# nihaomiao/CVPR23_LFDM

Measured on AMD Instinct MI355X. Metric: 40-frame 128x128 videos/sec (DDIM-100), higher is better.
Workload: dtype f32; 1 GPU; MUG 128x128, 40-frame DDIM-100 sample, batch=1 per GPU (BASELINE.json configs[1]); global_batch=1, frames=40, latent=32, image=128, sampler=DDIM-100 eta=1, cond_scale=1, parallelism=replicas x1 (videos sharded, no collective)

## Files before the change

cvpr23_lfdm_amd/csrc/attn_lowres.hip:

```cpp
#include <stdlib.h>

#include "attn_core.h"
#include "../../include/lfdm_hip.h"

namespace {

constexpr int NQ = 3 * DH;
constexpr int LDQ = NQ + 4;

template <int NT, int D>
__device__ __forceinline__ void project_wave_d(const float* __restrict__ x, int ldx, int64_t row0, int64_t rstride, int nrows,
                                               int c_begin, int c_end, const float* __restrict__ wf, int C, int head,
                                               f32x4 (&acc)[NT][6], float (&s1)[NT], float (&s2)[NT]) {
  const int lane = threadIdx.x & 63, l15 = lane & 15, ks = lane >> 4;
  const float* arow[NT];
#pragma unroll
  for (int ti = 0; ti < NT; ++ti) {
    int r = 16 * ti + l15;
    if (r >= nrows) r = nrows - 1;
    arow[ti] = x + (row0 + (int64_t)r * rstride) * ldx + 4 * ks;
    s1[ti] = s2[ti] = 0.f;
  }
  const float* brow[6];
#pragma unroll
  for (int nj = 0; nj < 6; ++nj) {
    const int gcol = (nj >> 1) * OUT_LD + head * DH + (nj & 1) * 16 + l15;
    brow[nj] = wf + (int64_t)gcol * C + 4 * ks;
#pragma unroll
    for (int ti = 0; ti < NT; ++ti) acc[ti][nj] = (f32x4){0.f, 0.f, 0.f, 0.f};
  }
  float4 ra[D][NT], rb[D][6];
  const int last = c_end - 16;
#pragma unroll
  for (int d = 0; d < D; ++d) {
    const int c = c_begin + 16 * d < last ? c_begin + 16 * d : last;
#pragma unroll
    for (int ti = 0; ti < NT; ++ti) ra[d][ti] = *reinterpret_cast<const float4*>(arow[ti] + c);
#pragma unroll
    for (int nj = 0; nj < 6; ++nj) rb[d][nj] = *reinterpret_cast<const float4*>(brow[nj] + c);
  }
  for (int c0 = c_begin; c0 < c_end; c0 += 16 * D) {
#pragma unroll
    for (int d = 0; d < D; ++d) {
      float4 a[NT], b[6];
#pragma unroll
      for (int ti = 0; ti < NT; ++ti) a[ti] = ra[d][ti];
#pragma unroll
      for (int nj = 0; nj < 6; ++nj) b[nj] = rb[d][nj];
      const int cn = c0 + 16 * (d + D) < last ? c0 + 16 * (d + D) : last;
#pragma unroll
      for (int ti = 0; ti < NT; ++ti) ra[d][ti] = *reinterpret_cast<const float4*>(arow[ti] + cn);
#pragma unroll
      for (int nj = 0; nj < 6; ++nj) rb[d][nj] = *reinterpret_cast<const float4*>(brow[nj] + cn);
#pragma unroll
      for (int ti = 0; ti < NT; ++ti) {
        s1[ti] += (a[ti].x + a[ti].y) + (a[ti].z + a[ti].w);
        s2[ti] += (a[ti].x * a[ti].x + a[ti].y * a[ti].y) + (a[ti].z * a[ti].z + a[ti].w * a[ti].w);
      }
#pragma unroll
      for (int nj = 0; nj < 6; ++nj)
#pragma unroll
        for (int ti = 0; ti < NT; ++ti) {
          acc[ti][nj] = mfma_16x16x4(a[ti].x, b[nj].x, acc[ti][nj]);
          acc[ti][nj] = mfma_16x16x4(a[ti].y, b[nj].y, acc[ti][nj]);
          acc[ti][nj] = mfma_16x16x4(a[ti].z, b[nj].z, acc[ti][nj]);
          acc[ti][nj] = mfma_16x16x4(a[ti].w, b[nj].w, acc[ti][nj]);
        }
    }
  }
#pragma unroll
  for (int ti = 0; ti < NT; ++ti) {
    s1[ti] += __shfl_xor(s1[ti], 16); s2[ti] += __shfl_xor(s2[ti], 16);
    s1[ti] += __shfl_xor(s1[ti], 32); s2[ti] += __shfl_xor(s2[ti], 32);
  }
}

template <int NT, int G, int D>
__device__ __forceinline__ void project_wave_asm(const float* __restrict__ x, int ldx, int64_t row0, int64_t rstride, int nrows,
                                                 int c_begin, const float* __restrict__ wf, int C, int head,
                                                 f32x4 (&acc)[NT][6], float (&s1)[NT], float (&s2)[NT]) {
  const int lane = threadIdx.x & 63, l15 = lane & 15, ks = lane >> 4;
  const float* arow[NT];
#pragma unroll
  for (int ti = 0; ti < NT; ++ti) {
    int r = 16 * ti + l15;
    if (r >= nrows) r = nrows - 1;
    arow[ti] = x + (row0 + (int64_t)r * rstride) * ldx + c_begin + 4 * ks;
    s1[ti] = s2[ti] = 0.f;
  }
  const float* brow[6];
#pragma unroll
  for (int nj = 0; nj < 6; ++nj) {
    const int gcol = (nj >> 1) * OUT_LD + head * DH + (nj & 1) * 16 + l15;
    brow[nj] = wf + (int64_t)gcol * C + c_begin + 4 * ks;
#pragma unroll
    for (int ti = 0; ti < NT; ++ti) acc[ti][nj] = (f32x4){0.f, 0.f, 0.f, 0.f};
  }
  f32x4 ra[D][NT], rb[D][6];
  auto issue = [&](auto gc) {
    constexpr int g = decltype(gc)::value, st = g % D;
    lfdm_static_for<0, NT>([&](auto ti) { lfdm_gload_f4<64 * g>(ra[st][decltype(ti)::value], arow[decltype(ti)::value]); });
    lfdm_static_for<0, 6>([&](auto nj) { lfdm_gload_f4<64 * g>(rb[st][decltype(nj)::value], brow[decltype(nj)::value]); });
  };
  lfdm_static_for<0, (D < G ? D : G)>(issue);
  lfdm_static_for<0, G>([&](auto gc) {
    constexpr int g = decltype(gc)::value, st = g % D;
    constexpr int younger = (G - 1 - g) < (D - 1) ? (G - 1 - g) : (D - 1);
    lfdm_vmwait<younger * (NT + 6)>();
#pragma unroll
    for (int ti = 0; ti < NT; ++ti) lfdm_tie(ra[st][ti]);
#pragma unroll
    for (int nj = 0; nj < 6; ++nj) lfdm_tie(rb[st][nj]);
    f32x4 a[NT], b[6];
#pragma unroll
    for (int ti = 0; ti < NT; ++ti) a[ti] = ra[st][ti];
#pragma unroll
    for (int nj = 0; nj < 6; ++nj) b[nj] = rb[st][nj];
    if constexpr (NT <= 2 && g + D < G) issue(std::integral_constant<int, g + D>{});
#pragma unroll
    for (int ti = 0; ti < NT; ++ti) {
      s1[ti] += (a[ti][0] + a[ti][1]) + (a[ti][2] + a[ti][3]);
      s2[ti] += (a[ti][0] * a[ti][0] + a[ti][1] * a[ti][1]) + (a[ti][2] * a[ti][2] + a[ti][3] * a[ti][3]);
    }
#pragma unroll
    for (int e = 0; e < 4; ++e)
#pragma unroll
      for (int nj = 0; nj < 6; ++nj)
#pragma unroll
        for (int ti = 0; ti < NT; ++ti) acc[ti][nj] = mfma_16x16x4(a[ti][e], b[nj][e], acc[ti][nj]);
    if constexpr (NT > 2 && g + D < G) issue(std::integral_constant<int, g + D>{});
  });
#pragma unroll
  for (int ti = 0; ti < NT; ++ti) {
    s1[ti] += __shfl_xor(s1[ti], 16); s2[ti] += __shfl_xor(s2[ti], 16);
    s1[ti] += __shfl_xor(s1[ti], 32); s2[ti] += __shfl_xor(s2[ti], 32);
  }
}

template <int NT, bool ASM = true>
__device__ __forceinline__ void project_wave(const float* __restrict__ x, int ldx, int64_t row0, int64_t rstride, int nrows,
                                             int c_begin, int c_end, const float* __restrict__ wf, int C, int head,
                                             f32x4 (&acc)[NT][6], float (&s1)[NT], float (&s2)[NT]) {
  const int groups = ASM ? (c_end - c_begin) >> 4 : 0;
  constexpr int D = NT == 1 ? 4 : 2;
  if (groups == 8) project_wave_asm<NT, 8, D>(x, ldx, row0, rstride, nrows, c_begin, wf, C, head, acc, s1, s2);
  else if (groups == 4) project_wave_asm<NT, 4, D>(x, ldx, row0, rstride, nrows, c_begin, wf, C, head, acc, s1, s2);
  else if (groups == 2) project_wave_asm<NT, 2, 2>(x, ldx, row0, rstride, nrows, c_begin, wf, C, head, acc, s1, s2);
  else project_wave_d<NT, 1>(x, ldx, row0, rstride, nrows, c_begin, c_end, wf, C, head, acc, s1, s2);
}

template <int NT, bool ASM = true>
__device__ __forceinline__ void project_ksplit(const float* __restrict__ x, int ldx, int64_t row0, int64_t rstride, int nrows,
                                               const float* __restrict__ wf, int C, int head, float eps, float* part,
                                               float* pstat, float* wsl, float wsum_val) {
  constexpr int R = 16 * NT;
  const int tid = threadIdx.x, lane = tid & 63, wave = tid >> 6, l15 = lane & 15, ks = lane >> 4;
  f32x4 acc[NT][6];
  float s1[NT], s2[NT];
  const int cw = C / 4;
  project_wave<NT, ASM>(x, ldx, row0, rstride, nrows, wave * cw, (wave + 1) * cw, wf, C, head, acc, s1, s2);
  float* mine = part + wave * (R * LDQ);
  if (tid < NQ) wsl[tid] = wsum_val;
#pragma unroll
  for (int ti = 0; ti < NT; ++ti) {
    if (ks == 0) {
      pstat[(0 * 4 + wave) * R + 16 * ti + l15] = s1[ti];
      pstat[(1 * 4 + wave) * R + 16 * ti + l15] = s2[ti];
    }
#pragma unroll
    for (int nj = 0; nj < 6; ++nj)
#pragma unroll
      for (int r = 0; r < 4; ++r) mine[(16 * ti + 4 * ks + r) * LDQ + 16 * nj + l15] = acc[ti][nj][r];
  }
  __syncthreads();
  const float inv_c = 1.0f / (float)C;
  for (int it = tid; it < R * (NQ / 4); it += 256) {
    const int row = it / (NQ / 4), q4 = it - row * (NQ / 4);
    float sv = 0.f, qv = 0.f;
#pragma unroll
    for (int w = 0; w < 4; ++w) {
      sv += pstat[(0 * 4 + w) * R + row];
      qv += pstat[(1 * 4 + w) * R + row];
    }
    const float mean = sv * inv_c;
    float var = qv * inv_c - mean * mean;
    if (var < 0.f) var = 0.f;
    const float rstd = 1.0f / sqrtf(var + eps);
    float4 v = *reinterpret_cast<const float4*>(part + row * LDQ + 4 * q4);
#pragma unroll
    for (int w = 1; w < 4; ++w) {
      const float4 u = *reinterpret_cast<const float4*>(part + w * (R * LDQ) + row * LDQ + 4 * q4);
      v.x += u.x; v.y += u.y; v.z += u.z; v.w += u.w;
    }
    const float4 ws = *reinterpret_cast<const float4*>(wsl + 4 * q4);
    v.x = rstd * (v.x - mean * ws.x); v.y = rstd * (v.y - mean * ws.y);
    v.z = rstd * (v.z - mean * ws.z); v.w = rstd * (v.w - mean * ws.w);
    *reinterpret_cast<float4*>(part + row * LDQ + 4 * q4) = v;
  }
  __syncthreads();
}

__device__ __forceinline__ float load_wsum(const float* __restrict__ wsum, int head) {
  const int tid = threadIdx.x;
  return tid < NQ ? wsum[(tid >> 5) * OUT_LD + head * DH + (tid & 31)] : 0.f;
}

template <int NT, bool MSPLIT>
__global__ __launch_bounds__(256) void linattn_lowres_kernel(const float* __restrict__ x, int ldx, int C,
                                                             const float* __restrict__ wf, const float* __restrict__ wsum,
                                                             float* __restrict__ out, int hw, float eps) {
  constexpr int R = 16 * NT;
  constexpr int ROWS = MSPLIT ? 4 * R : R;
  __shared__ __attribute__((aligned(16))) float qkv[(MSPLIT ? ROWS : 4 * R) * LDQ];
  __shared__ float pstat[2 * 4 * R];
  __shared__ __attribute__((aligned(16))) float wsl[NQ];
  __shared__ float red[8][DH], kmax[DH], ksum[DH];
  __shared__ __attribute__((aligned(16))) float ctx[DH][DH + 4];
  const int tid = threadIdx.x, lane = tid & 63, wave = tid >> 6, l15 = lane & 15, ks = lane >> 4;
  const int f = blockIdx.x >> 3, head = blockIdx.x & 7;
  const int64_t row0 = (int64_t)f * hw;
  const float wsum_val = load_wsum(wsum, head);

  if (MSPLIT) {
    f32x4 acc[NT][6];
    float s1[NT], s2[NT];
    const int nrows_w = hw - wave * R;
    project_wave<NT>(x, ldx, row0 + wave * R, 1, nrows_w < R ? nrows_w : R, 0, C, wf, C, head, acc, s1, s2);
    if (tid < NQ) wsl[tid] = wsum_val;
    if (ks == 0) {
#pragma unroll
      for (int ti = 0; ti < NT; ++ti) {
        const float mean = s1[ti] / (float)C;
        float var = s2[ti] / (float)C - mean * mean;
        if (var < 0.f) var = 0.f;
        pstat[wave * R + 16 * ti + l15] = mean;
        pstat[4 * R + wave * R + 16 * ti + l15] = 1.0f / sqrtf(var + eps);
      }
    }
    __syncthreads();
#pragma unroll
    for (int ti = 0; ti < NT; ++ti)
#pragma unroll
      for (int r = 0; r < 4; ++r) {
        const int rl = 16 * ti + 4 * ks + r;
        const float mean = pstat[wave * R + rl], rstd = pstat[4 * R + wave * R + rl];
#pragma unroll
        for (int nj = 0; nj < 6; ++nj)
          qkv[(wave * R + rl) * LDQ + 16 * nj + l15] = rstd * (acc[ti][nj][r] - mean * wsl[16 * nj + l15]);
      }
    __syncthreads();
  } else {
    project_ksplit<NT>(x, ldx, row0, 1, hw, wf, C, head, eps, qkv, pstat, wsl, wsum_val);
  }

  {
    const int d = tid & 31, part = tid >> 5;
    float m = -3.0e38f;
    for (int n = part; n < hw; n += 8) m = fmaxf(m, qkv[n * LDQ + DH + d]);
    red[part][d] = m;
    __syncthreads();
    if (tid < DH) {
      float mm = red[0][tid];
#pragma unroll
      for (int p = 1; p < 8; ++p) mm = fmaxf(mm, red[p][tid]);
      kmax[tid] = mm;
    }
    __syncthreads();
    const float mx = kmax[d];
    float s = 0.f;
    for (int n = part; n < hw; n += 8) {
      const float e = fast_exp(qkv[n * LDQ + DH + d] - mx);
      qkv[n * LDQ + DH + d] = e;
      s += e;
    }
    red[part][d] = s;
    __syncthreads();
    if (tid < DH) {
      float ss = 0.f;
#pragma unroll
      for (int p = 0; p < 8; ++p) ss += red[p][tid];
      ksum[tid] = ss;
    }
    __syncthreads();
  }
  {
    const int d = tid >> 3, e0 = (tid & 7) * 4;
    float a0 = 0.f, a1 = 0.f, a2 = 0.f, a3 = 0.f;
    for (int n = 0; n < hw; ++n) {
      const float e = qkv[n * LDQ + DH + d];
      const float4 v4 = *reinterpret_cast<const float4*>(qkv + n * LDQ + 2 * DH + e0);
      a0 = fmaf(e, v4.x, a0); a1 = fmaf(e, v4.y, a1); a2 = fmaf(e, v4.z, a2); a3 = fmaf(e, v4.w, a3);
    }
    const float ss = fast_rcp(ksum[d]);
    *reinterpret_cast<float4*>(&ctx[d][e0]) = make_float4(a0 * ss, a1 * ss, a2 * ss, a3 * ss);
  }
  for (int n0 = 0; n0 < hw; n0 += 32) {
    const bool live = n0 + (tid >> 3) < hw;
    const int n = live ? n0 + (tid >> 3) : hw - 1;
    float4 q4 = *reinterpret_cast<const float4*>(qkv + n * LDQ + 4 * (tid & 7));
    float m = fmaxf(fmaxf(q4.x, q4.y), fmaxf(q4.z, q4.w));
    m = fmaxf(m, __shfl_xor(m, 1)); m = fmaxf(m, __shfl_xor(m, 2)); m = fmaxf(m, __shfl_xor(m, 4));
    q4.x = fast_exp(q4.x - m); q4.y = fast_exp(q4.y - m); q4.z = fast_exp(q4.z - m); q4.w = fast_exp(q4.w - m);
    float s = (q4.x + q4.y) + (q4.z + q4.w);
    s += __shfl_xor(s, 1); s += __shfl_xor(s, 2); s += __shfl_xor(s, 4);
    s = ATT_SCALE * fast_rcp(s);
    q4.x *= s; q4.y *= s; q4.z *= s; q4.w *= s;
    if (live) *reinterpret_cast<float4*>(qkv + n * LDQ + 4 * (tid & 7)) = q4;
  }
  __syncthreads();
  for (int it = tid; it < hw * 8; it += 256) {
    const int n = it >> 3, e0 = (it & 7) * 4;
    float4 o = make_float4(0.f, 0.f, 0.f, 0.f);
#pragma unroll
    for (int d4 = 0; d4 < DH / 4; ++d4) {
      const float4 q4 = *reinterpret_cast<const float4*>(qkv + n * LDQ + 4 * d4);
      const float qd[4] = {q4.x, q4.y, q4.z, q4.w};
#pragma unroll
      for (int i = 0; i < 4; ++i) {
        const float4 c4 = *reinterpret_cast<const float4*>(&ctx[4 * d4 + i][e0]);
        o.x = fmaf(c4.x, qd[i], o.x); o.y = fmaf(c4.y, qd[i], o.y); o.z = fmaf(c4.z, qd[i], o.z); o.w = fmaf(c4.w, qd[i], o.w);
      }
    }
    *reinterpret_cast<float4*>(out + (row0 + n) * OUT_LD + head * DH + e0) = o;
  }
}

template <int NT>
__global__ __launch_bounds__(256) void attn_lowres_kernel(const float* __restrict__ x, int ldx, int C,
                                                          const float* __restrict__ wf, const float* __restrict__ wsum,
                                                          float* __restrict__ out, int frames, int hw, int mode,
                                                          const float* __restrict__ bias, const float* __restrict__ rot_cos,
                                                          const float* __restrict__ rot_sin, float eps) {
  constexpr int R = 16 * NT;
  __shared__ __attribute__((aligned(16))) float qkv[4 * R * LDQ];
  __shared__ float pstat[2 * 4 * R];
  __shared__ __attribute__((aligned(16))) float wsl[NQ];
  const int tid = threadIdx.x, lane = tid & 63, wave = tid >> 6, l15 = lane & 15, lq = lane >> 4;
  const int64_t unit = blockIdx.x;
  const int64_t seq = unit >> 3;
  const int head = (int)(unit & 7);
  int64_t row0, tstride;
  seq_rows(seq, mode, frames, hw, row0, tstride);
  const int L = mode == 0 ? frames : hw;
  const float wsum_val = load_wsum(wsum, head);
  project_ksplit<NT, (NT <= 3)>(x, ldx, row0, tstride, L, wf, C, head, eps, qkv, pstat, wsl, wsum_val);

  for (int ti = wave; ti < NT; ti += 4) {
    float qf[8], kf[NT][8];
    {
      const int t = ti * 16 + l15;
      const float* src = qkv + t * LDQ + 8 * lq;
      const float4 q0 = *reinterpret_cast<const float4*>(src), q1 = *reinterpret_cast<const float4*>(src + 4);
      qf[0] = q0.x * ATT_SCALE; qf[1] = q0.y * ATT_SCALE; qf[2] = q0.z * ATT_SCALE; qf[3] = q0.w * ATT_SCALE;
      qf[4] = q1.x * ATT_SCALE; qf[5] = q1.y * ATT_SCALE; qf[6] = q1.z * ATT_SCALE; qf[7] = q1.w * ATT_SCALE;
      if (rot_cos && t < L) {
#pragma unroll
        for (int pr = 0; pr < 4; ++pr) {
          const float c = rot_cos[t * 16 + 4 * lq + pr], sn = rot_sin[t * 16 + 4 * lq + pr];
          rot_pair(qf[2 * pr], qf[2 * pr + 1], c, sn);
        }
      }
    }
#pragma unroll
    for (int tj = 0; tj < NT; ++tj) {
      const int t = tj * 16 + l15;
      const float* src = qkv + t * LDQ + DH + 8 * lq;
      const float4 k0 = *reinterpret_cast<const float4*>(src), k1 = *reinterpret_cast<const float4*>(src + 4);
      kf[tj][0] = k0.x; kf[tj][1] = k0.y; kf[tj][2] = k0.z; kf[tj][3] = k0.w;
      kf[tj][4] = k1.x; kf[tj][5] = k1.y; kf[tj][6] = k1.z; kf[tj][7] = k1.w;
      if (rot_cos && t < L) {
#pragma unroll
        for (int pr = 0; pr < 4; ++pr) {
          const float c = rot_cos[t * 16 + 4 * lq + pr], sn = rot_sin[t * 16 + 4 * lq + pr];
          rot_pair(kf[tj][2 * pr], kf[tj][2 * pr + 1], c, sn);
        }
      }
    }
    f32x4 st[NT];
#pragma unroll
    for (int tj = 0; tj < NT; ++tj) {
      f32x4 a = {0.f, 0.f, 0.f, 0.f};
#pragma unroll
      for (int s = 0; s < 8; ++s) a = mfma_16x16x4(kf[tj][s], qf[s], a);
      st[tj] = a;
    }
    const float inv = softmax_tile<NT, true>(st, head, L, ti * 16 + l15, lq, bias, false);
    f32x4 o0 = {0.f, 0.f, 0.f, 0.f}, o1 = o0;
#pragma unroll
    for (int tj = 0; tj < NT; ++tj)
#pragma unroll
      for (int r = 0; r < 4; ++r) {
        const float p = st[tj][r] * inv;
        const float* vr = qkv + (16 * tj + 4 * lq + r) * LDQ + 2 * DH;
        o0 = mfma_16x16x4(p, vr[l15], o0);
        o1 = mfma_16x16x4(p, vr[16 + l15], o1);
      }
#pragma unroll
    for (int r = 0; r < 4; ++r) {
      const int t = ti * 16 + lq * 4 + r;
      if (t < L) {
        float* dst = out + (row0 + (int64_t)t * tstride) * OUT_LD + head * DH;
        dst[l15] = o0[r];
        dst[16 + l15] = o1[r];
      }
    }
  }
}

bool lowres_args_ok(const float* x, int ldx, int channels, const float* wqkv, const float* wsum, const float* out) {
  return x && wqkv && wsum && out && channels >= 64 && channels % 64 == 0 && ldx >= channels && ldx % 4 == 0 &&
         ((((uintptr_t)x) | ((uintptr_t)wqkv) | ((uintptr_t)out)) & 15) == 0;
}

}

extern "C" int lfdm_linear_attention_lowres_cl_f32(const float* x, int ldx, int channels, const float* wqkv, const float* wsum,
                                                   float* out, int n_frames, int hw, float ln_eps, lfdm_stream_t stream_) {
  hipStream_t stream = (hipStream_t)stream_;
  if (!lowres_args_ok(x, ldx, channels, wqkv, wsum, out) || n_frames <= 0 || hw <= 0 || hw > 256 || (int64_t)n_frames * HEADS > 0x7fffffff) {
    lfdm_set_error("linear_attention_lowres: needs C % 64 == 0, 1 <= hw <= 256 pixels per frame, 16-byte aligned rows");
    return LFDM_EINVAL;
  }
  const dim3 grid((unsigned)(n_frames * HEADS)), block(256);
  if (hw > 192) LFDM_LAUNCH((linattn_lowres_kernel<4, true>), grid, block, 0, stream, x, ldx, channels, wqkv, wsum, out, hw, ln_eps);
  else if (hw > 64) {
    lfdm_set_error("linear_attention_lowres: 64 < hw <= 192 pixels per frame is not built (use the unfused entry points)");
    return LFDM_EINVAL;
  } else
    lfdm_ladder<16, 32, 64>(hw, [&](auto rows) {
      LFDM_LAUNCH((linattn_lowres_kernel<decltype(rows)::value / 16, false>), grid, block, 0, stream, x, ldx, channels, wqkv, wsum, out, hw, ln_eps);
    });
  return lfdm_check_launch("linear_attention_lowres");
}

extern "C" int lfdm_attention_lowres_cl_f32(const float* x, int ldx, int channels, const float* wqkv, const float* wsum,
                                            float* out, int batch, int frames, int hw, int mode, const float* bias,
                                            const float* rot_cos, const float* rot_sin, float ln_eps, lfdm_stream_t stream_) {
  hipStream_t stream = (hipStream_t)stream_;
  const int L = mode == 0 ? frames : hw;
  const int64_t nseq = mode == 0 ? (int64_t)batch * hw : (int64_t)batch * frames;
  if (!lowres_args_ok(x, ldx, channels, wqkv, wsum, out) || batch <= 0 || frames <= 0 || hw <= 0 || (mode != 0 && mode != 1) || L > 64 ||
      ((rot_cos == nullptr) != (rot_sin == nullptr)) || nseq * HEADS > 0x7fffffff) {
    lfdm_set_error("attention_lowres: needs C % 64 == 0, <= 64 tokens per sequence, 16-byte aligned rows");
    return LFDM_EINVAL;
  }
  const dim3 grid((unsigned)(nseq * HEADS)), block(256);
  lp_ladder(L, [&](auto lp) {
    LFDM_LAUNCH((attn_lowres_kernel<decltype(lp)::value / 16>), grid, block, 0, stream, x, ldx, channels, wqkv, wsum, out, frames, hw, mode, bias, rot_cos, rot_sin, ln_eps);
  });
  return lfdm_check_launch("attention_lowres");
}
```

cvpr23_lfdm_amd/csrc/lfdm_device.h:

```cpp
#pragma once
#include <stddef.h>
#include <stdint.h>
#include <type_traits>

#if defined(LFDM_EMU_BUILD)
#include "hip_emu.h"
typedef emu_f32x16 f32x16;
typedef emu_f32x4 f32x4;
#define LFDM_LAUNCH(kern, grid, block, smem, stream, ...) \
  emu::launch(grid, block, smem, [=]() { kern(__VA_ARGS__); })
static inline f32x16 mfma_32x32x2(float a, float b, f32x16 c) { return emu_mfma_32x32x2(a, b, c); }
static inline f32x4 mfma_16x16x4(float a, float b, f32x4 c) { return emu_mfma_16x16x4(a, b, c); }
static inline f32x4 mfma_4x4x1(float a, float b, f32x4 c) { return emu_mfma_4x4x1(a, b, c); }
struct lfdm_bf16x8 { uint16_t h[8]; };
static inline uint16_t lfdm_f32_to_bf16(float f) {
  uint32_t u;
  memcpy(&u, &f, 4);
  if ((u & 0x7fffffffu) > 0x7f800000u) return (uint16_t)((u >> 16) | 0x40u);
  u += 0x7fffu + ((u >> 16) & 1u);
  return (uint16_t)(u >> 16);
}
static inline float lfdm_bf16_to_f32(uint16_t h) {
  const uint32_t u = (uint32_t)h << 16;
  float f;
  memcpy(&f, &u, 4);
  return f;
}
static inline lfdm_bf16x8 lfdm_cvt_bf16x8(float4 a0, float4 a1) {
  const float f[8] = {a0.x, a0.y, a0.z, a0.w, a1.x, a1.y, a1.z, a1.w};
  lfdm_bf16x8 r;
  for (int i = 0; i < 8; ++i) r.h[i] = lfdm_f32_to_bf16(f[i]);
  return r;
}
static inline uint32_t lfdm_cvt_pk_bf16(float lo, float hi) { return (uint32_t)lfdm_f32_to_bf16(lo) | ((uint32_t)lfdm_f32_to_bf16(hi) << 16); }
static inline lfdm_bf16x8 lfdm_bf16x8_bits(float4 v) {
  lfdm_bf16x8 r;
  memcpy(&r, &v, 16);
  return r;
}
static inline f32x16 mfma_32x32x16_bf16(lfdm_bf16x8 a, lfdm_bf16x8 b, f32x16 c) {
  struct Pair { lfdm_bf16x8 a, b; };
  struct Whole { lfdm_bf16x8 a[2], b[2]; };
  const unsigned lane = emu::lane_id(), h = lane >> 5;
  const Pair other = emu::wave_read_from(Pair{a, b}, lane ^ 32u);
  Whole mine;
  mine.a[h] = a;
  mine.a[1 - h] = other.a;
  mine.b[h] = b;
  mine.b[1 - h] = other.b;
  for (int r = 0; r < 16; ++r) {
    const unsigned row = (r & 3) + 8 * (r >> 2) + 4 * h;
    const Whole src = emu::wave_read_from(mine, row);
    float acc = c[r];
    for (int k = 0; k < 16; ++k)
      acc = fmaf(lfdm_bf16_to_f32(src.a[k >> 3].h[k & 7]), lfdm_bf16_to_f32(mine.b[k >> 3].h[k & 7]), acc);
    c[r] = acc;
  }
  return c;
}
#else
#include <hip/hip_runtime.h>
typedef float f32x16 __attribute__((ext_vector_type(16)));
typedef float f32x4 __attribute__((ext_vector_type(4)));
#define LFDM_LAUNCH(kern, grid, block, smem, stream, ...) \
  hipLaunchKernelGGL(kern, grid, block, smem, stream, __VA_ARGS__)
__device__ __forceinline__ f32x16 mfma_32x32x2(float a, float b, f32x16 c) {
  return __builtin_amdgcn_mfma_f32_32x32x2f32(a, b, c, 0, 0, 0);
}
__device__ __forceinline__ f32x4 mfma_16x16x4(float a, float b, f32x4 c) {
  return __builtin_amdgcn_mfma_f32_16x16x4f32(a, b, c, 0, 0, 0);
}
__device__ __forceinline__ f32x4 mfma_4x4x1(float a, float b, f32x4 c) {
  return __builtin_amdgcn_mfma_f32_4x4x1f32(a, b, c, 0, 0, 0);
}
typedef __bf16 lfdm_bf16x8 __attribute__((ext_vector_type(8)));
typedef __bf16 lfdm_bf16x2 __attribute__((ext_vector_type(2)));
typedef float lfdm_f32x8 __attribute__((ext_vector_type(8)));
typedef float lfdm_f32x2 __attribute__((ext_vector_type(2)));
__device__ __forceinline__ lfdm_bf16x8 lfdm_cvt_bf16x8(float4 a0, float4 a1) {
  const lfdm_f32x8 f = {a0.x, a0.y, a0.z, a0.w, a1.x, a1.y, a1.z, a1.w};
  return __builtin_convertvector(f, lfdm_bf16x8);
}
__device__ __forceinline__ uint32_t lfdm_cvt_pk_bf16(float lo, float hi) {
  const lfdm_f32x2 f = {lo, hi};
  return __builtin_bit_cast(uint32_t, __builtin_convertvector(f, lfdm_bf16x2));
}
__device__ __forceinline__ lfdm_bf16x8 lfdm_bf16x8_bits(float4 v) { return __builtin_bit_cast(lfdm_bf16x8, v); }
__device__ __forceinline__ f32x16 mfma_32x32x16_bf16(lfdm_bf16x8 a, lfdm_bf16x8 b, f32x16 c) {
  return __builtin_amdgcn_mfma_f32_32x32x16_bf16(a, b, c, 0, 0, 0);
}
#endif

#define LFDM_WAVE 64

template <int BEGIN, int END, class F>
__device__ __forceinline__ void lfdm_static_for(F&& f) {
  if constexpr (BEGIN < END) {
    f(std::integral_constant<int, BEGIN>{});
    lfdm_static_for<BEGIN + 1, END>(f);
  }
}

#if defined(LFDM_EMU_BUILD)
struct lfdm_buf {
  const char* base;
  uint32_t bytes;
};
static inline lfdm_buf lfdm_make_buf(const void* p, uint32_t bytes) { return lfdm_buf{(const char*)p, bytes}; }
static inline float4 lfdm_buf_load_f4(lfdm_buf b, uint32_t off) {
  float4 v = make_float4(0.f, 0.f, 0.f, 0.f);
  if ((uint64_t)off + 16u <= (uint64_t)b.bytes) memcpy(&v, b.base + off, 16);
  return v;
}
static inline float2 lfdm_buf_load_f2(lfdm_buf b, uint32_t off) {
  float2 v = make_float2(0.f, 0.f);
  if ((uint64_t)off + 8u <= (uint64_t)b.bytes) memcpy(&v, b.base + off, 8);
  return v;
}
#else
typedef __amdgpu_buffer_rsrc_t lfdm_buf;
typedef int lfdm_i32x4 __attribute__((ext_vector_type(4)));
__device__ __forceinline__ lfdm_buf lfdm_make_buf(const void* p, uint32_t bytes) {
  return __builtin_amdgcn_make_buffer_rsrc(const_cast<void*>(p), 0, (int)bytes, 0x00020000);
}
__device__ __forceinline__ float4 lfdm_buf_load_f4(lfdm_buf b, uint32_t off) {
  const lfdm_i32x4 v = __builtin_amdgcn_raw_buffer_load_b128(b, (int)off, 0, 0);
  float4 f;
  f.x = __int_as_float(v.x);
  f.y = __int_as_float(v.y);
  f.z = __int_as_float(v.z);
  f.w = __int_as_float(v.w);
  return f;
}
typedef int lfdm_i32x2 __attribute__((ext_vector_type(2)));
__device__ __forceinline__ float2 lfdm_buf_load_f2(lfdm_buf b, uint32_t off) {
  const lfdm_i32x2 v = __builtin_amdgcn_raw_buffer_load_b64(b, (int)off, 0, 0);
  return make_float2(__int_as_float(v.x), __int_as_float(v.y));
}
#endif
#define LFDM_BUF_OOB 0xFFFFFFF0u

#if defined(LFDM_EMU_BUILD)
static inline void lfdm_buf_store_f4_sc1(lfdm_buf b, uint32_t off, float4 v) {
  if ((uint64_t)off + 16u <= (uint64_t)b.bytes) memcpy(const_cast<char*>(b.base) + off, &v, 16);
}
static inline float4 lfdm_buf_load_f4_sc1(lfdm_buf b, uint32_t off) { return lfdm_buf_load_f4(b, off); }
#else
__device__ __forceinline__ void lfdm_buf_store_f4_sc1(lfdm_buf b, uint32_t off, float4 v) {
  lfdm_i32x4 d;
  d.x = __float_as_int(v.x); d.y = __float_as_int(v.y); d.z = __float_as_int(v.z); d.w = __float_as_int(v.w);
  __builtin_amdgcn_raw_buffer_store_b128(d, b, (int)off, 0, 16);
}
__device__ __forceinline__ float4 lfdm_buf_load_f4_sc1(lfdm_buf b, uint32_t off) {
  const lfdm_i32x4 v = __builtin_amdgcn_raw_buffer_load_b128(b, (int)off, 0, 16);
  float4 f;
  f.x = __int_as_float(v.x); f.y = __int_as_float(v.y); f.z = __int_as_float(v.z); f.w = __int_as_float(v.w);
  return f;
}
#endif

#if defined(LFDM_EMU_BUILD)
template <int OFF = 0> static inline void lfdm_gload_f4(f32x4& dst, const float* p) { memcpy(&dst, (const char*)p + OFF, 16); }
template <int N> static inline void lfdm_vmwait() {}
template <int N> static inline void lfdm_vmwait(f32x4&) {}
template <int N> static inline void lfdm_vmwait(f32x4&, f32x4&) {}
template <int N> static inline void lfdm_vmwait(f32x4&, f32x4&, f32x4&, f32x4&) {}
static inline void lfdm_tie(f32x4&) {}
static inline int lfdm_uniform(int v) { return v; }
#else
template <int OFF = 0>
__device__ __forceinline__ void lfdm_gload_f4(f32x4& dst, const float* p) {
  asm volatile("global_load_dwordx4 %0, %1, off offset:%2" : "=v"(dst) : "v"(p), "n"(OFF) : "memory");
}
template <int N> __device__ __forceinline__ void lfdm_vmwait() { asm volatile("s_waitcnt vmcnt(%0)" ::"n"(N) : "memory"); }
template <int N> __device__ __forceinline__ void lfdm_vmwait(f32x4& a) { asm volatile("s_waitcnt vmcnt(%1)" : "+v"(a) : "n"(N) : "memory"); }
template <int N> __device__ __forceinline__ void lfdm_vmwait(f32x4& a, f32x4& b) {
  asm volatile("s_waitcnt vmcnt(%2)" : "+v"(a), "+v"(b) : "n"(N) : "memory");
}
template <int N> __device__ __forceinline__ void lfdm_vmwait(f32x4& a, f32x4& b, f32x4& c, f32x4& d) {
  asm volatile("s_waitcnt vmcnt(%4)" : "+v"(a), "+v"(b), "+v"(c), "+v"(d) : "n"(N) : "memory");
}
__device__ __forceinline__ void lfdm_tie(f32x4& a) { asm volatile("" : "+v"(a)::"memory"); }
__device__ __forceinline__ int lfdm_uniform(int v) { return __builtin_amdgcn_readfirstlane(v); }
#endif

#if defined(LFDM_EMU_BUILD)
#define LFDM_DRAIN_STORES() ((void)0)
#define LFDM_FENCE_RELEASE_AGENT() ((void)0)
#define LFDM_FENCE_ACQUIRE_AGENT() ((void)0)
static inline unsigned lfdm_ticket_take(unsigned* c) { return __atomic_fetch_add(c, 1u, __ATOMIC_SEQ_CST); }
static inline void lfdm_ticket_reset(unsigned* c) { __atomic_store_n(c, 0u, __ATOMIC_SEQ_CST); }
#else
#define LFDM_DRAIN_STORES() asm volatile("s_waitcnt vmcnt(0)" ::: "memory")
#define LFDM_FENCE_RELEASE_AGENT() __builtin_amdgcn_fence(__ATOMIC_RELEASE, "agent")
#define LFDM_FENCE_ACQUIRE_AGENT() __builtin_amdgcn_fence(__ATOMIC_ACQUIRE, "agent")
__device__ __forceinline__ unsigned lfdm_ticket_take(unsigned* c) {
  return __hip_atomic_fetch_add(c, 1u, __ATOMIC_RELAXED, __HIP_MEMORY_SCOPE_AGENT);
}
__device__ __forceinline__ void lfdm_ticket_reset(unsigned* c) {
  __hip_atomic_store(c, 0u, __ATOMIC_RELAXED, __HIP_MEMORY_SCOPE_AGENT);
}
#endif

#if defined(__HIP_DEVICE_COMPILE__) && !defined(__gfx950__) && !defined(LFDM_EMU_BUILD)
#error "fence-free hand-off (lfdm_agent_store_u64 / lfdm_agent_load_u64 / lfdm_ticket_take) validated on gfx950 only: re-validate, or use LFDM_FENCE_RELEASE_AGENT / LFDM_FENCE_ACQUIRE_AGENT, before building for another target"
#endif
#if defined(LFDM_EMU_BUILD)
static inline void lfdm_agent_store_u64(unsigned long long* p, unsigned long long v) { __atomic_store_n(p, v, __ATOMIC_SEQ_CST); }
static inline unsigned long long lfdm_agent_load_u64(const unsigned long long* p) { return __atomic_load_n(p, __ATOMIC_SEQ_CST); }
static inline unsigned lfdm_agent_load_u32(const unsigned* p) { return __atomic_load_n(p, __ATOMIC_SEQ_CST); }
static inline void lfdm_sleep() {}
#else
__device__ __forceinline__ void lfdm_agent_store_u64(unsigned long long* p, unsigned long long v) {
  __hip_atomic_store(p, v, __ATOMIC_RELAXED, __HIP_MEMORY_SCOPE_AGENT);
}
__device__ __forceinline__ unsigned long long lfdm_agent_load_u64(const unsigned long long* p) {
  return __hip_atomic_load(p, __ATOMIC_RELAXED, __HIP_MEMORY_SCOPE_AGENT);
}
__device__ __forceinline__ unsigned lfdm_agent_load_u32(const unsigned* p) { return __hip_atomic_load(p, __ATOMIC_RELAXED, __HIP_MEMORY_SCOPE_AGENT); }
__device__ __forceinline__ void lfdm_sleep() { __builtin_amdgcn_s_sleep(2); }
#endif

#if defined(LFDM_EMU_BUILD)
static inline void lfdm_wave_lds_sync() { emu::wave_sync(); }
#else
__device__ __forceinline__ void lfdm_wave_lds_sync() {
  __builtin_amdgcn_fence(__ATOMIC_RELEASE, "wavefront");
  __builtin_amdgcn_wave_barrier();
  __builtin_amdgcn_fence(__ATOMIC_ACQUIRE, "wavefront");
}
#endif

__device__ __forceinline__ float wave_sum(float v) {
#pragma unroll
  for (int m = 32; m >= 1; m >>= 1) v += __shfl_xor(v, m);
  return v;
}
__device__ __forceinline__ float wave_max(float v) {
#pragma unroll
  for (int m = 32; m >= 1; m >>= 1) v = fmaxf(v, __shfl_xor(v, m));
  return v;
}
#if defined(LFDM_EMU_BUILD)
static inline float fast_exp(float x) { return expf(x); }
static inline float fast_rcp(float x) { return 1.0f / x; }
#else
__device__ __forceinline__ float fast_exp(float x) { return __expf(x); }
__device__ __forceinline__ float fast_rcp(float x) { return __builtin_amdgcn_rcpf(x); }
#endif
__device__ __forceinline__ float sigmoidf_(float x) { return 1.0f / (1.0f + expf(-x)); }
__device__ __forceinline__ float siluf_(float x) { return x / (1.0f + expf(-x)); }

#if defined(LFDM_EMU_BUILD)
static inline float silu_fast_(float x) { return x / (1.0f + expf(-x)); }
#else
__device__ __forceinline__ float silu_fast_(float x) { return x * __builtin_amdgcn_rcpf(1.0f + __expf(-x)); }
#endif

#if defined(LFDM_TUNING_KNOBS) || defined(LFDM_EMU_BUILD)
static inline const char* lfdm_knob(const char* name) { return getenv(name); }
#else
static inline const char* lfdm_knob(const char*) { return nullptr; }
#endif

__device__ __forceinline__ float apply_act(float v, int act) {
  if (act == 1) return v > 0.f ? v : 0.f;
  if (act == 2) return sigmoidf_(v);
  if (act == 3) return siluf_(v);
  return v;
}

extern "C" void lfdm_set_error(const char* msg);
int lfdm_check_launch(const char* what);
```

Measured before the change: 4.128 videos/s.

## Add register-lean SGPR-addressed projection path with staged k-split reduction for NT=4

For the NT=4 low-res attention kernel, the QKV projection now uses scalar base pointers with 32-bit VGPR offsets (global_load with saddr). It also adds sched barriers around the MFMA block and a short runtime loop of 2-group pipelines. The k-split partials are reduced through two shared tiles in staged adds instead of four, which halves LDS use. Launch bounds request 2 blocks per CU. The aim is to cut VGPR and LDS pressure so two workgroups fit per CU and overlap better, at the cost of extra syncthreads and reduction passes.

```diff
diff --git a/cvpr23_lfdm_amd/csrc/attn_lowres.hip b/cvpr23_lfdm_amd/csrc/attn_lowres.hip
--- a/cvpr23_lfdm_amd/csrc/attn_lowres.hip
+++ b/cvpr23_lfdm_amd/csrc/attn_lowres.hip
@@ -75,6 +75,47 @@
   }
 }
 
+template <int NT, int G, int D, bool TIGHT, class LA, class LB>
+__device__ __forceinline__ void asm_pipeline(LA load_a, LB load_b, f32x4 (&acc)[NT][6], float (&s1)[NT], float (&s2)[NT]) {
+  f32x4 ra[D][NT], rb[D][6];
+  auto issue = [&](auto gc) {
+    constexpr int g = decltype(gc)::value, st = g % D;
+    lfdm_static_for<0, NT>([&](auto ti) { load_a(ra[st][decltype(ti)::value], ti, gc); });
+    lfdm_static_for<0, 6>([&](auto nj) { load_b(rb[st][decltype(nj)::value], nj, gc); });
+  };
+  lfdm_static_for<0, (D < G ? D : G)>(issue);
+  lfdm_static_for<0, G>([&](auto gc) {
+    constexpr int g = decltype(gc)::value, st = g % D;
+    constexpr int younger = (G - 1 - g) < (D - 1) ? (G - 1 - g) : (D - 1);
+    lfdm_vmwait<younger * (NT + 6)>();
+#pragma unroll
+    for (int ti = 0; ti < NT; ++ti) lfdm_tie(ra[st][ti]);
+#pragma unroll
+    for (int nj = 0; nj < 6; ++nj) lfdm_tie(rb[st][nj]);
+    f32x4 a[NT], b[6];
+#pragma unroll
+    for (int ti = 0; ti < NT; ++ti) a[ti] = ra[st][ti];
+#pragma unroll
+    for (int nj = 0; nj < 6; ++nj) b[nj] = rb[st][nj];
+    if constexpr (NT <= 2 && g + D < G) issue(std::integral_constant<int, g + D>{});
+#pragma unroll
+    for (int ti = 0; ti < NT; ++ti) {
+      s1[ti] += (a[ti][0] + a[ti][1]) + (a[ti][2] + a[ti][3]);
+      s2[ti] += (a[ti][0] * a[ti][0] + a[ti][1] * a[ti][1]) + (a[ti][2] * a[ti][2] + a[ti][3] * a[ti][3]);
+    }
+    if constexpr (TIGHT) lfdm_sched_fence();
+#pragma unroll
+    for (int e = 0; e < 4; ++e)
+#pragma unroll
+      for (int nj = 0; nj < 6; ++nj)
+#pragma unroll
+        for (int ti = 0; ti < NT; ++ti) acc[ti][nj] = mfma_16x16x4(a[ti][e], b[nj][e], acc[ti][nj]);
+    if constexpr (TIGHT) lfdm_sched_fence();
+    if constexpr (NT > 2 && g + D < G) issue(std::integral_constant<int, g + D>{});
+    if constexpr (TIGHT) lfdm_sched_fence();
+  });
+}
+
 template <int NT, int G, int D>
 __device__ __forceinline__ void project_wave_asm(const float* __restrict__ x, int ldx, int64_t row0, int64_t rstride, int nrows,
                                                  int c_begin, const float* __restrict__ wf, int C, int head,
@@ -96,40 +137,9 @@
 #pragma unroll
     for (int ti = 0; ti < NT; ++ti) acc[ti][nj] = (f32x4){0.f, 0.f, 0.f, 0.f};
   }
-  f32x4 ra[D][NT], rb[D][6];
-  auto issue = [&](auto gc) {
-    constexpr int g = decltype(gc)::value, st = g % D;
-    lfdm_static_for<0, NT>([&](auto ti) { lfdm_gload_f4<64 * g>(ra[st][decltype(ti)::value], arow[decltype(ti)::value]); });
-    lfdm_static_for<0, 6>([&](auto nj) { lfdm_gload_f4<64 * g>(rb[st][decltype(nj)::value], brow[decltype(nj)::value]); });
-  };
-  lfdm_static_for<0, (D < G ? D : G)>(issue);
-  lfdm_static_for<0, G>([&](auto gc) {
-    constexpr int g = decltype(gc)::value, st = g % D;
-    constexpr int younger = (G - 1 - g) < (D - 1) ? (G - 1 - g) : (D - 1);
-    lfdm_vmwait<younger * (NT + 6)>();
-#pragma unroll
-    for (int ti = 0; ti < NT; ++ti) lfdm_tie(ra[st][ti]);
-#pragma unroll
-    for (int nj = 0; nj < 6; ++nj) lfdm_tie(rb[st][nj]);
-    f32x4 a[NT], b[6];
-#pragma unroll
-    for (int ti = 0; ti < NT; ++ti) a[ti] = ra[st][ti];
-#pragma unroll
-    for (int nj = 0; nj < 6; ++nj) b[nj] = rb[st][nj];
-    if constexpr (NT <= 2 && g + D < G) issue(std::integral_constant<int, g + D>{});
-#pragma unroll
-    for (int ti = 0; ti < NT; ++ti) {
-      s1[ti] += (a[ti][0] + a[ti][1]) + (a[ti][2] + a[ti][3]);
-      s2[ti] += (a[ti][0] * a[ti][0] + a[ti][1] * a[ti][1]) + (a[ti][2] * a[ti][2] + a[ti][3] * a[ti][3]);
-    }
-#pragma unroll
-    for (int e = 0; e < 4; ++e)
-#pragma unroll
-      for (int nj = 0; nj < 6; ++nj)
-#pragma unroll
-        for (int ti = 0; ti < NT; ++ti) acc[ti][nj] = mfma_16x16x4(a[ti][e], b[nj][e], acc[ti][nj]);
-    if constexpr (NT > 2 && g + D < G) issue(std::integral_constant<int, g + D>{});
-  });
+  asm_pipeline<NT, G, D, false>(
+      [&](f32x4& dst, auto ti, auto gc) { lfdm_gload_f4<64 * decltype(gc)::value>(dst, arow[decltype(ti)::value]); },
+      [&](f32x4& dst, auto nj, auto gc) { lfdm_gload_f4<64 * decltype(gc)::value>(dst, brow[decltype(nj)::value]); }, acc, s1, s2);
 #pragma unroll
   for (int ti = 0; ti < NT; ++ti) {
     s1[ti] += __shfl_xor(s1[ti], 16); s2[ti] += __shfl_xor(s2[ti], 16);
@@ -137,10 +147,60 @@
   }
 }
 
-template <int NT, bool ASM = true>
+template <int NT>
+__device__ __forceinline__ void project_wave_tight(const float* __restrict__ x, int ldx, int64_t row0, int64_t rstride, int nrows,
+                                                   int c_begin, int c_end, const float* __restrict__ wf, int C, int head,
+                                                   f32x4 (&acc)[NT][6], float (&s1)[NT], float (&s2)[NT]) {
+  const int lane = threadIdx.x & 63, l15 = lane & 15, ks = lane >> 4;
+#pragma unroll
+  for (int ti = 0; ti < NT; ++ti) {
+    s1[ti] = s2[ti] = 0.f;
+#pragma unroll
+    for (int nj = 0; nj < 6; ++nj) acc[ti][nj] = (f32x4){0.f, 0.f, 0.f, 0.f};
+  }
+  const float* abase = x + lfdm_uniform64(row0 * ldx + c_begin);
+  const float* bbase[6];
+  unsigned aoff[NT];
+  const unsigned rpitch = (unsigned)rstride * (unsigned)ldx * 4u;
+#pragma unroll
+  for (int ti = 0; ti < NT; ++ti) {
+    int r = 16 * ti + l15;
+    if (r >= nrows) r = nrows - 1;
+    unsigned rb = (unsigned)r * rpitch;
+    lfdm_tie(rb);
+    aoff[ti] = rb + 16u * (unsigned)ks;
+  }
+#pragma unroll
+  for (int nj = 0; nj < 6; ++nj)
+    bbase[nj] = wf + lfdm_uniform64((int64_t)((nj >> 1) * OUT_LD + head * DH + (nj & 1) * 16) * C + c_begin);
+  const unsigned boff = ((unsigned)l15 * (unsigned)C + 4u * (unsigned)ks) * 4u;
+  auto load_a = [&](f32x4& dst, auto ti, auto gc) { lfdm_gload_f4_s<64 * decltype(gc)::value>(dst, aoff[decltype(ti)::value], abase); };
+  auto load_b = [&](f32x4& dst, auto nj, auto gc) { lfdm_gload_f4_s<64 * decltype(gc)::value>(dst, boff, bbase[decltype(nj)::value]); };
+  const int groups = (c_end - c_begin) >> 4;
+  if (groups == 4) {
+    asm_pipeline<NT, 4, 2, true>(load_a, load_b, acc, s1, s2);
+  } else {
+#pragma nounroll
+    for (int h = 0; h < (groups >> 1); ++h) {
+      asm_pipeline<NT, 2, 2, true>(load_a, load_b, acc, s1, s2);
+      abase += 32;
+#pragma unroll
+      for (int nj = 0; nj < 6; ++nj) bbase[nj] += 32;
+    }
+    if (groups & 1) asm_pipeline<NT, 1, 2, true>(load_a, load_b, acc, s1, s2);
+  }
+#pragma unroll
+  for (int ti = 0; ti < NT; ++ti) {
+    s1[ti] += __shfl_xor(s1[ti], 16); s2[ti] += __shfl_xor(s2[ti], 16);
+    s1[ti] += __shfl_xor(s1[ti], 32); s2[ti] += __shfl_xor(s2[ti], 32);
+  }
+}
+
+template <int NT, bool ASM = true, bool TIGHT = false>
 __device__ __forceinline__ void project_wave(const float* __restrict__ x, int ldx, int64_t row0, int64_t rstride, int nrows,
                                              int c_begin, int c_end, const float* __restrict__ wf, int C, int head,
                                              f32x4 (&acc)[NT][6], float (&s1)[NT], float (&s2)[NT]) {
+  if constexpr (TIGHT) return project_wave_tight<NT>(x, ldx, row0, rstride, nrows, c_begin, c_end, wf, C, head, acc, s1, s2);
   const int groups = ASM ? (c_end - c_begin) >> 4 : 0;
   constexpr int D = NT == 1 ? 4 : 2;
   if (groups == 8) project_wave_asm<NT, 8, D>(x, ldx, row0, rstride, nrows, c_begin, wf, C, head, acc, s1, s2);
@@ -149,7 +209,10 @@
   else project_wave_d<NT, 1>(x, ldx, row0, rstride, nrows, c_begin, c_end, wf, C, head, acc, s1, s2);
 }
 
-template <int NT, bool ASM = true>
+template <bool STAGED>
+constexpr int KSPLIT_TILES = STAGED ? 2 : 4;
+
+template <int NT, bool ASM = true, bool STAGED = false>
 __device__ __forceinline__ void project_ksplit(const float* __restrict__ x, int ldx, int64_t row0, int64_t rstride, int nrows,
                                                const float* __restrict__ wf, int C, int head, float eps, float* part,
                                                float* pstat, float* wsl, float wsum_val) {
@@ -158,8 +221,9 @@
   f32x4 acc[NT][6];
   float s1[NT], s2[NT];
   const int cw = C / 4;
-  project_wave<NT, ASM>(x, ldx, row0, rstride, nrows, wave * cw, (wave + 1) * cw, wf, C, head, acc, s1, s2);
-  float* mine = part + wave * (R * LDQ);
+  const int c_first = STAGED ? lfdm_uniform(wave * cw) : wave * cw;
+  project_wave<NT, ASM, STAGED>(x, ldx, row0, rstride, nrows, c_first, c_first + cw, wf, C, head, acc, s1, s2);
+  float* mine = part + (STAGED ? wave >> 1 : wave) * (R * LDQ);
   if (tid < NQ) wsl[tid] = wsum_val;
 #pragma unroll
   for (int ti = 0; ti < NT; ++ti) {
@@ -167,12 +231,40 @@
       pstat[(0 * 4 + wave) * R + 16 * ti + l15] = s1[ti];
       pstat[(1 * 4 + wave) * R + 16 * ti + l15] = s2[ti];
     }
-#pragma unroll
-    for (int nj = 0; nj < 6; ++nj)
-#pragma unroll
-      for (int r = 0; r < 4; ++r) mine[(16 * ti + 4 * ks + r) * LDQ + 16 * nj + l15] = acc[ti][nj][r];
+    if (!STAGED || (wave & 1)) {
+#pragma unroll
+      for (int nj = 0; nj < 6; ++nj)
+#pragma unroll
+        for (int r = 0; r < 4; ++r) mine[(16 * ti + 4 * ks + r) * LDQ + 16 * nj + l15] = acc[ti][nj][r];
+    }
   }
   __syncthreads();
+  if (STAGED) {
+    if (wave == 0) {
+#pragma unroll
+      for (int ti = 0; ti < NT; ++ti)
+#pragma unroll
+        for (int nj = 0; nj < 6; ++nj)
+#pragma unroll
+          for (int r = 0; r < 4; ++r) {
+            float* p = part + (16 * ti + 4 * ks + r) * LDQ + 16 * nj + l15;
+            *p = acc[ti][nj][r] + *p;
+          }
+    }
+    __syncthreads();
+    if (wave == 2) {
+#pragma unroll
+      for (int ti = 0; ti < NT; ++ti)
+#pragma unroll
+        for (int nj = 0; nj < 6; ++nj)
+#pragma unroll
+          for (int r = 0; r < 4; ++r) {
+            float* p = part + (16 * ti + 4 * ks + r) * LDQ + 16 * nj + l15;
+            *p = *p + acc[ti][nj][r];
+          }
+    }
+    __syncthreads();
+  }
   const float inv_c = 1.0f / (float)C;
   for (int it = tid; it < R * (NQ / 4); it += 256) {
     const int row = it / (NQ / 4), q4 = it - row * (NQ / 4);
@@ -188,7 +280,7 @@
     const float rstd = 1.0f / sqrtf(var + eps);
     float4 v = *reinterpret_cast<const float4*>(part + row * LDQ + 4 * q4);
 #pragma unroll
-    for (int w = 1; w < 4; ++w) {
+    for (int w = 1; w < KSPLIT_TILES<STAGED>; ++w) {
       const float4 u = *reinterpret_cast<const float4*>(part + w * (R * LDQ) + row * LDQ + 4 * q4);
       v.x += u.x; v.y += u.y; v.z += u.z; v.w += u.w;
     }
@@ -206,12 +298,13 @@
 }
 
 template <int NT, bool MSPLIT>
-__global__ __launch_bounds__(256) void linattn_lowres_kernel(const float* __restrict__ x, int ldx, int C,
+__global__ __launch_bounds__(256, (NT == 4 && !MSPLIT) ? 2 : 1) void linattn_lowres_kernel(const float* __restrict__ x, int ldx, int C,
                                                              const float* __restrict__ wf, const float* __restrict__ wsum,
                                                              float* __restrict__ out, int hw, float eps) {
   constexpr int R = 16 * NT;
   constexpr int ROWS = MSPLIT ? 4 * R : R;
-  __shared__ __attribute__((aligned(16))) float qkv[(MSPLIT ? ROWS : 4 * R) * LDQ];
+  constexpr bool STAGED = NT == 4;
+  __shared__ __attribute__((aligned(16))) float qkv[(MSPLIT ? ROWS : KSPLIT_TILES<STAGED> * R) * LDQ];
   __shared__ float pstat[2 * 4 * R];
   __shared__ __attribute__((aligned(16))) float wsl[NQ];
   __shared__ float red[8][DH], kmax[DH], ksum[DH];
@@ -250,7 +343,7 @@
       }
     __syncthreads();
   } else {
-    project_ksplit<NT>(x, ldx, row0, 1, hw, wf, C, head, eps, qkv, pstat, wsl, wsum_val);
+    project_ksplit<NT, true, STAGED>(x, ldx, row0, 1, hw, wf, C, head, eps, qkv, pstat, wsl, wsum_val);
   }
 
   {
@@ -417,8 +510,9 @@
 extern "C" int lfdm_linear_attention_lowres_cl_f32(const float* x, int ldx, int channels, const float* wqkv, const float* wsum,
                                                    float* out, int n_frames, int hw, float ln_eps, lfdm_stream_t stream_) {
   hipStream_t stream = (hipStream_t)stream_;
-  if (!lowres_args_ok(x, ldx, channels, wqkv, wsum, out) || n_frames <= 0 || hw <= 0 || hw > 256 || (int64_t)n_frames * HEADS > 0x7fffffff) {
-    lfdm_set_error("linear_attention_lowres: needs C % 64 == 0, 1 <= hw <= 256 pixels per frame, 16-byte aligned rows");
+  if (!lowres_args_ok(x, ldx, channels, wqkv, wsum, out) || n_frames <= 0 || hw <= 0 || hw > 256 || (int64_t)n_frames * HEADS > 0x7fffffff ||
+      ldx >= (1 << 24)) {
+    lfdm_set_error("linear_attention_lowres: needs C % 64 == 0, 1 <= hw <= 256 pixels per frame, 16-byte aligned rows of fewer than 2^24 floats");
     return LFDM_EINVAL;
   }
   const dim3 grid((unsigned)(n_frames * HEADS)), block(256);
diff --git a/cvpr23_lfdm_amd/csrc/lfdm_device.h b/cvpr23_lfdm_amd/csrc/lfdm_device.h
--- a/cvpr23_lfdm_amd/csrc/lfdm_device.h
+++ b/cvpr23_lfdm_amd/csrc/lfdm_device.h
@@ -166,7 +166,11 @@
 template <int N> static inline void lfdm_vmwait(f32x4&, f32x4&) {}
 template <int N> static inline void lfdm_vmwait(f32x4&, f32x4&, f32x4&, f32x4&) {}
 static inline void lfdm_tie(f32x4&) {}
+static inline void lfdm_tie(unsigned&) {}
 static inline int lfdm_uniform(int v) { return v; }
+static inline int64_t lfdm_uniform64(int64_t v) { return v; }
+template <int OFF = 0> static inline void lfdm_gload_f4_s(f32x4& dst, unsigned off, const float* base) { memcpy(&dst, (const char*)base + off + OFF, 16); }
+static inline void lfdm_sched_fence() {}
 #else
 template <int OFF = 0>
 __device__ __forceinline__ void lfdm_gload_f4(f32x4& dst, const float* p) {
@@ -181,7 +185,17 @@
   asm volatile("s_waitcnt vmcnt(%4)" : "+v"(a), "+v"(b), "+v"(c), "+v"(d) : "n"(N) : "memory");
 }
 __device__ __forceinline__ void lfdm_tie(f32x4& a) { asm volatile("" : "+v"(a)::"memory"); }
+__device__ __forceinline__ void lfdm_tie(unsigned& a) { asm volatile("" : "+v"(a)); }
 __device__ __forceinline__ int lfdm_uniform(int v) { return __builtin_amdgcn_readfirstlane(v); }
+__device__ __forceinline__ int64_t lfdm_uniform64(int64_t v) {
+  const unsigned lo = __builtin_amdgcn_readfirstlane((int)(unsigned)v), hi = __builtin_amdgcn_readfirstlane((int)(v >> 32));
+  return (int64_t)(((uint64_t)hi << 32) | lo);
+}
+template <int OFF = 0>
+__device__ __forceinline__ void lfdm_gload_f4_s(f32x4& dst, unsigned off, const float* base) {
+  asm volatile("global_load_dwordx4 %0, %1, %2 offset:%3" : "=v"(dst) : "v"(off), "s"(base), "n"(OFF) : "memory");
+}
+__device__ __forceinline__ void lfdm_sched_fence() { __builtin_amdgcn_sched_barrier(0); }
 #endif
 
 #if defined(LFDM_EMU_BUILD)
```

New measurement: 4.150 videos/s, median of 6. About the same (+0.5%).
